# yamatokataoka/reinforcement-learning-replications

Measured on NVIDIA H100. Metric: ppo_update_transitions_per_sec, higher is better.
Workload: dtype f32

## Files before the change

### reinforcement-learning-replications_b200/csrc/mlp_tc3.cu

```cuda
#include <cuda_fp16.h>

#include <cmath>

#include "common.cuh"
#include "policy_head.cuh"
#include "tc2_common.cuh"
#include "tc_common.cuh"
#include "tc3.cuh"

namespace b200rl {

constexpr int T3_ROWS = 128;
constexpr int T3_CHAIN_WARPS = 8;
constexpr int T3_THREADS = T3_CHAIN_WARPS * 32 + 256;
constexpr int T3_WARPS = T3_THREADS / 32;

constexpr uint32_t S3_XB = 0;
constexpr uint32_t S3_H1 = 2 * T2_ACT;
constexpr uint32_t S3_H2 = S3_H1 + 2 * T2_ACT;
constexpr uint32_t S3_DZ2 = S3_H2 + 2 * T2_ACT;
constexpr uint32_t S3_DZ1 = S3_DZ2 + 2 * T2_ACT;
constexpr uint32_t T3_W1T = 32 * 128, T3_W2 = 64 * 128, T3_W3 = 16 * 128;
constexpr uint32_t S3_DO = S3_DZ1 + 2 * T2_ACT;
constexpr uint32_t S3_W = S3_DO + T2_ACT;
constexpr uint32_t S3_WNET = 2 * T3_W1T + 2 * T3_W2 + 2 * T3_W3;
constexpr uint32_t S3_OPERANDS_END = S3_W + S3_WNET;
constexpr uint32_t S3_BIAS = S3_OPERANDS_END;
constexpr uint32_t S3_DIST = S3_BIAS + 2 * 640;
constexpr uint32_t S3_SCALE = S3_DIST + 256;
constexpr uint32_t S3_XS = S3_SCALE + 128;
constexpr uint32_t S3_ADV = S3_XS + 256;
constexpr uint32_t S3_RED = S3_ADV + 16;
constexpr uint32_t S3_BARS = S3_RED + 4 * 8 * T3_WARPS;
constexpr uint32_t T3_LI_IN = 15 * T3_ROWS, T3_LI_OLD = 16 * T3_ROWS;
constexpr uint32_t T3_LI_BYTES = 17 * T3_ROWS * 4;
constexpr uint32_t S3_LOSS = S3_BARS + 128;
constexpr uint32_t S3_TOTAL = S3_LOSS + 2 * T3_LI_BYTES;
constexpr uint32_t T3_SMEM_BYTES = S3_TOTAL + 1024;
static_assert(T3_SMEM_BYTES <= 227 * 1024, "mlp_tc3 shared memory");
constexpr uint32_t S3_END_DB3 = 0;
constexpr uint32_t S3_END_SC = 1024;

constexpr uint32_t ACC_GRAD_NET = 176;
constexpr uint32_t ACC_DB3 = 2 * ACC_GRAD_NET;
static_assert(ACC_DB3 + 4 * 16 <= ACC_COLS, "mlp_tc3 accumulator columns");
constexpr uint32_t ACC_DW2 = 0, ACC_DB2 = 64, ACC_DW1 = 80, ACC_DW3 = 144;

__device__ __forceinline__ uint32_t grad_acc_off(uint32_t pcol, int n, int row, int col) {
  const int rr = row & 63;
  const int t = 32 * (rr >> 4) + 4 * (rr & 7) + ((col >> 1) & 3);
  const int e = 2 * ((rr >> 3) & 1) + (col & 1);
  return pcol * ACC_LANES + (uint32_t)((row >> 6) * 64 * n + 4 * (128 * (col >> 3) + t) + e);
}

#ifdef B200RL_TC3_TIMING
__device__ unsigned long long g_tc3_t[64];
#endif

enum { C3_G = 0, C3_U1, C3_U2, C3_U3, C3_UH2, C3_UH1, C3_W1, C3_W2, C3_W3, C3_OW3, C3_OW2, C3_OW1, C3_OB, C3_N };

__device__ __forceinline__ void mbar_arrive_expect_tx(uint32_t bar, uint32_t bytes) {
  asm volatile("mbarrier.arrive.expect_tx.shared::cta.b64 _, [%0], %1;" ::"r"(bar), "r"(bytes) : "memory");
}
__device__ __forceinline__ void bulk_copy_g2s(uint32_t dst_smem, const void* src, uint32_t bytes, uint32_t bar) {
  asm volatile("cp.async.bulk.shared::cluster.global.mbarrier::complete_tx::bytes [%0], [%1], %2, [%3];" ::"r"(dst_smem),
               "l"(src), "r"(bytes), "r"(bar)
               : "memory");
}

__global__ void __launch_bounds__(128) pack_obs_kernel(const float* __restrict__ obs, long long n_rows, int n_in,
                                                       const float* __restrict__ absmax, uint8_t* __restrict__ ximg,
                                                       float* __restrict__ xscale, float* __restrict__ bad_flag) {
  __shared__ float s_xs[32];
  const int r = threadIdx.x;
  bool bad = false;
  if (r < 32) {
    const int e = r < n_in ? fit_exp(__ldg(absmax + r), bad) : 0;
    s_xs[r] = pow2i(e);
    if (blockIdx.x == 0) {
      xscale[r] = pow2i(e);
      xscale[32 + r] = pow2i(-e);
    }
  }
  __syncthreads();
  const long long tiles = (n_rows + T3_ROWS - 1) / T3_ROWS;
  for (long long t = blockIdx.x; t < tiles; t += gridDim.x) {
    const long long row = t * T3_ROWS + r;
    float x[32];
#pragma unroll
    for (int c = 0; c < 32; ++c) x[c] = 0.f;
    if (row < n_rows) {
      const float* src = obs + row * n_in;
      float rmax = 0.f, probe = 0.f;
#pragma unroll
      for (int c = 0; c < 31; ++c)
        if (c < n_in) {
          x[c] = __ldg(src + c) * s_xs[c];
          rmax = fmaxf(rmax, fabsf(x[c]));
          probe += x[c];
        }
      if (!(rmax <= T2_RANGE) || probe != probe) bad = true;
      if (rmax > 0.f && rmax < 0.03125f) bad = true;
      x[31] = 1.0f;
    }
    uint4 h[4], l[4];
#pragma unroll
    for (int j = 0; j < 4; ++j) {
      split2h(x[8 * j + 0], x[8 * j + 1], h[j].x, l[j].x);
      split2h(x[8 * j + 2], x[8 * j + 3], h[j].y, l[j].y);
      split2h(x[8 * j + 4], x[8 * j + 5], h[j].z, l[j].z);
      split2h(x[8 * j + 6], x[8 * j + 7], h[j].w, l[j].w);
    }
    uint8_t* dst = ximg + (size_t)t * T2_ACT + (size_t)r * 128;
#pragma unroll
    for (int j = 0; j < 4; ++j) {
      *reinterpret_cast<uint4*>(dst + ((j ^ (r & 7)) << 4)) = h[j];
      *reinterpret_cast<uint4*>(dst + (((4 + j) ^ (r & 7)) << 4)) = l[j];
    }
  }
  if (bad) *bad_flag = 1.0f;
}

template <int N, int TA, int TB, int TERMS, int KSTEPS>
__device__ __forceinline__ void wg_mma(float (&d)[N / 2], const uint32_t (&alo)[TERMS], const uint32_t (&blo)[TERMS],
                                       uint32_t a_hi, uint32_t b_hi, uint32_t a_k, uint32_t b_k, uint32_t accumulate) {
  wgmma_fence();
#pragma unroll
  for (int s = 0; s < TERMS; ++s)
#pragma unroll
    for (int k = 0; k < KSTEPS; ++k)
      wgmma_run<N, TA, TB>(d, ((uint64_t)a_hi << 32) | (alo[s] + (uint32_t)k * a_k),
                           ((uint64_t)b_hi << 32) | (blo[s] + (uint32_t)k * b_k), s == 0 && k == 0 ? accumulate : 1u);
  wgmma_commit();
  wgmma_wait_all();
}
template <int N, int TB, int KSTEPS>
__device__ __forceinline__ void chain_mma(float (&d)[N / 2], const Op2 a, const Op2 b) {
  const uint32_t alo[3] = {a.lo, a.lo + a.split_step, a.lo}, blo[3] = {b.lo + b.split_step, b.lo, b.lo};
#pragma unroll
  for (int i = 0; i < N / 2; ++i) d[i] = 0.f;
  wg_mma<N, K_MAJOR, TB, 3, KSTEPS>(d, alo, blo, a.hi, b.hi, a.k_step, b.k_step, 0u);
}
__device__ __forceinline__ void stmatrix_x4(uint32_t addr, const uint32_t (&r)[4]) {
  asm volatile("stmatrix.sync.aligned.m8n8.x4.shared.b16 [%0], {%1, %2, %3, %4};" ::"r"(addr), "r"(r[0]), "r"(r[1]),
               "r"(r[2]), "r"(r[3])
               : "memory");
}
__device__ __forceinline__ void ldmatrix_x4(uint32_t addr, uint32_t (&r)[4]) {
  asm volatile("ldmatrix.sync.aligned.m8n8.x4.shared.b16 {%0, %1, %2, %3}, [%4];"
               : "=r"(r[0]), "=r"(r[1]), "=r"(r[2]), "=r"(r[3])
               : "r"(addr)
               : "memory");
}
__device__ __forceinline__ float* grad_frag(float* acc_cta, uint32_t pcol) {
  const int t = (int)(threadIdx.x & 127u);
  return acc_cta + grad_acc_off(pcol, 0, 16 * (t >> 5) + ((t & 31) >> 2), 2 * (t & 3));
}
template <int N, int KSTEPS, int TERMS>
__device__ __forceinline__ void grad_products(float (&d)[N / 2], uint32_t a_lo, const Op2 a, const Op2 b, bool first) {
  uint32_t b_lo = b.lo;
  asm volatile("" : "+r"(a_lo), "+r"(b_lo));
#pragma unroll
  for (int s = 0; s < TERMS; ++s)
#pragma unroll
    for (int k = 0; k < KSTEPS; ++k)
      wgmma_run<N, MN_MAJOR, MN_MAJOR>(d, ((uint64_t)a.hi << 32) | (a_lo + (uint32_t)k * a.k_step),
                                       ((uint64_t)b.hi << 32) | (b_lo + (s + 1 < TERMS ? b.split_step : 0u) +
                                                                 (uint32_t)k * b.k_step),
                                       s == 0 && k == 0 ? (first ? 0u : 1u) : 1u);
}
template <int N>
__device__ __forceinline__ void grad_store(float* acc_cta, uint32_t pcol, int h, const float (&d)[N / 2]) {
  float* const frag = grad_frag(acc_cta, pcol) + 64 * N * h;
#pragma unroll
  for (int j = 0; j < N / 8; ++j)
    *reinterpret_cast<float4*>(frag + 512 * j) = make_float4(d[4 * j], d[4 * j + 1], d[4 * j + 2], d[4 * j + 3]);
}

__global__ void __launch_bounds__(T3_THREADS, 1) mlp_tc3_kernel(const Tc3Args p) {
  extern __shared__ uint8_t smem_raw[];
  const bool two = p.run_policy != 0 && p.run_value != 0;
  const int G = two ? (int)(gridDim.x >> 1) : (int)gridDim.x;
  const int c = two ? (int)blockIdx.x / G : (p.run_policy != 0 ? 0 : 1);
  const int slot = (int)blockIdx.x - c * (two ? G : 0);
  const bool run_p = p.run_policy != 0 && (p.stop_flag == nullptr || *p.stop_flag == 0);
  const bool run_v = p.run_value != 0;
  if (!(c == 0 ? run_p : run_v)) return;
  if (*p.x_bad != 0.f) return;
  const int tid = threadIdx.x, lane = tid & 31;
  float* const acc = p.acc_mem + (size_t)slot * ACC_CTA_FLOATS;
  const int warp = __shfl_sync(0xffffffffu, tid >> 5, 0);
  const uint32_t raw = smem_u32(smem_raw);
  const uint32_t base = (raw + 1023u) & ~1023u;
  uint8_t* sm = smem_raw + (base - raw);
  float* s_bias = reinterpret_cast<float*>(sm + S3_BIAS);
  float* s_dist = reinterpret_cast<float*>(sm + S3_DIST);
  float* s_scale = reinterpret_cast<float*>(sm + S3_SCALE);
  float* s_xs = reinterpret_cast<float*>(sm + S3_XS);
  float* s_adv = reinterpret_cast<float*>(sm + S3_ADV);
  float* s_red = reinterpret_cast<float*>(sm + S3_RED);
  int* s_bad = reinterpret_cast<int*>(sm + S3_BARS + 120);
  const uint32_t bars = base + S3_BARS;
  const int n_in = p.n_in;
  bool bad = false;
#ifdef B200RL_TC3_TIMING
  unsigned long long tacc[64];
  for (int i = 0; i < 64; ++i) tacc[i] = 0;
  const long long t_kernel0 = clock64();
#endif

  for (uint32_t i = S3_W / 16 + tid; i < S3_OPERANDS_END / 16; i += T3_THREADS) reinterpret_cast<uint4*>(sm)[i] = make_uint4(0, 0, 0, 0);
  if (tid == 0) {
    *s_bad = 0;
    float adv_mean, adv_std;
    adv_mean_std(p.adv_stats, adv_mean, adv_std);
    s_adv[0] = adv_mean;
    s_adv[1] = 1.f / adv_std;
  }
  if (tid < 64) s_xs[tid] = __ldg(p.xscale + tid);
  float* s_par = reinterpret_cast<float*>(sm + S3_H1);
  static_assert(S3_W - S3_H1 >= 4 * (2 * 6000 + 64), "parameter staging area");
#pragma unroll 1
  for (int net = 0; net < 2; ++net) {
    const float* par = p.params[net];
    float* dst = s_par + (net == 0 ? 0 : p.P[0]);
#pragma unroll 8
    for (int i = tid; i < p.P[net]; i += T3_THREADS) dst[i] = (*(par + i));
  }
  __syncthreads();
#pragma unroll 1
  for (int net = 0; net < 2; ++net) {
    const Tc3Net& nn = p.net[net];
    const float* par = s_par + (net == 0 ? 0 : p.P[0]);
    float m1 = 0.f, m2 = 0.f, m3 = 0.f;
    for (int idx = tid; idx < nn.h1 * n_in; idx += T3_THREADS) {
      const float w = (*(par + nn.w_off[0] + idx)) * s_xs[32 + idx % n_in];
      m1 = fmaxf(m1, fabsf(w));
      if (w != w) bad = true;
    }
    for (int idx = tid; idx < nn.h2 * nn.h1; idx += T3_THREADS) {
      const float w = (*(par + nn.w_off[1] + idx));
      m2 = fmaxf(m2, fabsf(w));
      if (w != w) bad = true;
    }
    for (int idx = tid; idx < nn.n_out * nn.h2; idx += T3_THREADS) {
      const float w = (*(par + nn.w_off[2] + idx));
      m3 = fmaxf(m3, fabsf(w));
      if (w != w) bad = true;
    }
#pragma unroll
    for (int o = 16; o > 0; o >>= 1) {
      m1 = fmaxf(m1, __shfl_xor_sync(0xffffffffu, m1, o));
      m2 = fmaxf(m2, __shfl_xor_sync(0xffffffffu, m2, o));
      m3 = fmaxf(m3, __shfl_xor_sync(0xffffffffu, m3, o));
    }
    if (lane == 0) {
      s_red[warp * 8 + 4 * net + 0] = m1;
      s_red[warp * 8 + 4 * net + 1] = m2;
      s_red[warp * 8 + 4 * net + 2] = m3;
    }
  }
  __syncthreads();
  if (bad) *s_bad = 1;
  bad = false;
  if (tid < 2) {
    const int net = tid;
    const Tc3Net& nn = p.net[net];
    float m1 = 0.f, m2 = 0.f, m3 = 0.f;
    for (int w = 0; w < T3_WARPS; ++w) {
      m1 = fmaxf(m1, s_red[w * 8 + 4 * net + 0]);
      m2 = fmaxf(m2, s_red[w * 8 + 4 * net + 1]);
      m3 = fmaxf(m3, s_red[w * 8 + 4 * net + 2]);
    }
    bool b0 = false;
    const int ew1 = fit_exp(m1, b0), ew2 = fit_exp(m2, b0), ew3 = fit_exp(m3, b0);
    float typ;
    if (net == 1) {
      const float tm = __ldg(p.target_absmax);
      typ = (tm > 0.f && tm < INFINITY) ? 0.25f * tm : 1.f;
    } else if (p.dist == B200RL_DIST_GAUSSIAN) {
      float smin = INFINITY;
      for (int a = 0; a < nn.n_out; ++a) smin = fminf(smin, expf(__ldg(p.log_std + a)));
      typ = (smin > 0.f && smin < INFINITY) ? 1.f / smin : 1.f;
    } else {
      typ = 0.5f;
    }
    int eg = 3 + ilogbf(p.n_glob_f) - ilogbf(typ);
    eg = eg < -100 ? -100 : (eg > 100 ? 100 : eg);
    float* sc = s_scale + 16 * net;
    sc[C3_G] = pow2i(eg);
    sc[C3_U1] = pow2i(-ew1);
    sc[C3_U2] = pow2i(-(T2_H_EXP + ew2));
    sc[C3_U3] = pow2i(-(T2_H_EXP + ew3));
    sc[C3_UH2] = pow2i(-ew3);
// ... 29 lines not shown
        put(wb + 2 * T3_W1T, T3_W2, idx / nn.h1, idx % nn.h1, (*(par + nn.w_off[1] + idx)) * sw2);
      for (int idx = tid; idx < nn.n_out * nn.h2; idx += T3_THREADS)
        put(wb + 2 * T3_W1T + 2 * T3_W2, T3_W3, idx / nn.h2, idx % nn.h2, (*(par + nn.w_off[2] + idx)) * sw3);
    }
    float* bb = s_bias + 160 * net;
    for (int i = tid; i < 64; i += T3_THREADS) {
      bb[i] = i < nn.h1 ? (*(par + nn.b_off[0] + i)) : 0.f;
      bb[64 + i] = i < nn.h2 ? (*(par + nn.b_off[1] + i)) : 0.f;
      if (!(fabsf(bb[i]) < INFINITY) || !(fabsf(bb[64 + i]) < INFINITY)) bad = true;
    }
    for (int i = tid; i < 16; i += T3_THREADS) {
      bb[128 + i] = i < nn.n_out ? (*(par + nn.b_off[2] + i)) : 0.f;
      if (!(fabsf(bb[128 + i]) < INFINITY)) bad = true;
    }
  }
  if (p.dist == B200RL_DIST_GAUSSIAN)
    for (int a = tid; a < p.net[0].n_out; a += T3_THREADS) {
      const NormalConsts nc = normal_consts(p.log_std, a);
      s_dist[a] = nc.var;
      s_dist[16 + a] = nc.log_scale;
      s_dist[32 + a] = nc.inv_2var;
      s_dist[48 + a] = nc.inv_var;
    }
  if (bad) *s_bad = 1;
  bad = false;
  if (tid == 0) {
    mbar_init(bars + 0, 1);
    mbar_init(bars + 8, 1);
    for (int i = 0; i < 3; ++i) {
      mbar_init(bars + 16 + 8 * i, 2);
      mbar_init(bars + 40 + 8 * i, 2);
    }
    fence_mbar_init();
  }
  fence_proxy_async_smem();
  __syncthreads();

  const long long num_tiles = (p.n_rows + T3_ROWS - 1) / T3_ROWS;
  const int cta_tiles = (int)((num_tiles - slot + G - 1) / G);

  constexpr int K = K_MAJOR, MN = MN_MAJOR;
  const uint32_t ub = base;
  auto bar_ready = [&](int s) { return bars + 16u + 8u * (uint32_t)(s - 3); };
  auto bar_done = [&](int s) { return bars + 40u + 8u * (uint32_t)(s - 3); };
  double sc[5] = {0, 0, 0, 0, 0};
  int rows_done = 0;
#ifdef B200RL_TC3_TIMING
  long long t_loop0 = 0, t_loop_end = 0;
#endif

  if (warp >= T3_CHAIN_WARPS) {
    const Op2 X_M = op2_mnmajor(ub + S3_XB, T2_ACT, 64);
    const Op2 X_M16 = op2_mnmajor(ub + S3_XB + 32, T2_ACT, 64);
    const Op2 DO_M = op2_at(op2_mnmajor(ub + S3_DO, T2_ACT, 32), c * 64);
    const Op2 H1_M = op2_mnmajor(ub + S3_H1, T2_ACT, T2_ACT), H2_M = op2_mnmajor(ub + S3_H2, T2_ACT, T2_ACT);
    const Op2 DZ2_M = op2_mnmajor(ub + S3_DZ2, T2_ACT, T2_ACT), DZ1_M = op2_mnmajor(ub + S3_DZ1, T2_ACT, T2_ACT);
    const int g = (warp - T3_CHAIN_WARPS) >> 2;
    const bool producer = g == 0;
    const uint32_t ah = (uint32_t)g * (T2_ACT >> 4);
    const uint32_t gcol = c * ACC_GRAD_NET;
    float w3[16], w2[32], b2[8], w1[32];
    const uint32_t act_bytes = T3_ROWS * 4u * (uint32_t)(p.dist == B200RL_DIST_GAUSSIAN ? p.net[0].n_out : 1);
    auto load_x = [&](int k) {
      const uint32_t b = (uint32_t)(k & 1), bar = bars + 8 * b;
      const long long tile = slot + (long long)k * G;
      const size_t row0 = (size_t)tile * T3_ROWS;
      const uint32_t li = ub + S3_LOSS + b * T3_LI_BYTES;
      uint32_t e;
      asm volatile("{\n\t.reg .pred q;\n\telect.sync _|q, 0xffffffff;\n\tselp.u32 %0, 1, 0, q;\n\t}" : "=r"(e));
      if (e && (warp & 3) == 0) {
        if (c == 0) {
          mbar_arrive_expect_tx(bar, T2_ACT + act_bytes + 2 * T3_ROWS * 4);
          bulk_copy_g2s(li, reinterpret_cast<const uint8_t*>(p.actions) + (size_t)tile * act_bytes, act_bytes, bar);
          bulk_copy_g2s(li + 4 * T3_LI_IN, p.adv_raw + row0, T3_ROWS * 4, bar);
          bulk_copy_g2s(li + 4 * T3_LI_OLD, p.old_logp + row0, T3_ROWS * 4, bar);
        } else {
          mbar_arrive_expect_tx(bar, T2_ACT + T3_ROWS * 4);
          bulk_copy_g2s(li + 4 * T3_LI_IN, p.target + row0, T3_ROWS * 4, bar);
        }
        bulk_copy_g2s(ub + S3_XB + b * T2_ACT, p.ximg + (size_t)tile * T2_ACT, T2_ACT, bar);
      }
      __syncwarp();
    };
    auto release = [&](int stage) {
      wgmma_commit();
      wgmma_wait_all();
      asm volatile("bar.sync %0, 128;" ::"r"(8 + g) : "memory");
      if ((tid & 127) == 0) mbar_arrive(bar_done(stage));
    };
    if (producer && cta_tiles > 0) load_x(0);
#pragma unroll 1
    for (int k = 0; k < cta_tiles; ++k) {
      const uint32_t xo = (uint32_t)(k & 1) * T2_ACT;
      const bool first = k == 0;
      if (producer && k + 1 < cta_tiles) {
        if (k > 0) mbar_wait(bar_done(5), (uint32_t)((k - 1) & 1));
        load_x(k + 1);
      }
#ifdef B200RL_TC3_TIMING
      long long it0 = clock64(), it1;
#define TC3_GSPLIT(s)                                                   \
  it1 = clock64();                                                      \
  tacc[40 + 3 * g + (s) - 3] += (unsigned long long)(it1 - it0);
#define TC3_GEND(s)                                                     \
  it0 = clock64();                                                      \
  tacc[46 + 3 * g + (s) - 3] += (unsigned long long)(it0 - it1);
#else
#define TC3_GSPLIT(s)
#define TC3_GEND(s)
#endif
      mbar_wait(bar_ready(3), (uint32_t)(k & 1));
      TC3_GSPLIT(3)
      wgmma_fence();
      grad_products<32, 8, 1>(w3, H2_M.lo + ah, H2_M, DO_M, first);
      release(3);
      TC3_GEND(3)
      mbar_wait(bar_ready(4), (uint32_t)(k & 1));
      TC3_GSPLIT(4)
      wgmma_fence();
      grad_products<64, 8, 2>(w2, DZ2_M.lo + ah, DZ2_M, H1_M, first);
      grad_products<16, 8, 1>(b2, DZ2_M.lo + ah, DZ2_M, op2_at(X_M16, xo), first);
      release(4);
      TC3_GEND(4)
      mbar_wait(bar_ready(5), (uint32_t)(k & 1));
      TC3_GSPLIT(5)
      wgmma_fence();
      grad_products<64, 8, 1>(w1, DZ1_M.lo + ah, DZ1_M, op2_at(X_M, xo), first);
      release(5);
      TC3_GEND(5)
#undef TC3_GSPLIT
#undef TC3_GEND
    }
    if (cta_tiles > 0) {
      grad_store<32>(acc, gcol + ACC_DW3, g, w3);
      grad_store<64>(acc, gcol + ACC_DW2, g, w2);
      grad_store<16>(acc, gcol + ACC_DB2, g, b2);
      grad_store<64>(acc, gcol + ACC_DW1, g, w1);
    }
#ifdef B200RL_TC3_TIMING
    if ((tid & 127) == 0 && blockIdx.x == 0) {
      for (int s = 0; s < 3; ++s) {
        g_tc3_t[40 + 3 * g + s] = tacc[40 + 3 * g + s];
        g_tc3_t[46 + 3 * g + s] = tacc[46 + 3 * g + s];
      }
      if (producer) g_tc3_t[52] = (unsigned long long)cta_tiles;
    }
#endif
  } else {
    const int wg = warp >> 2;
    const int quad = lane >> 2, q = lane & 3;
    const int r0 = 64 * wg + 16 * (warp & 3) + quad;
    const uint32_t rows = (uint32_t)wg * (64u * 128u);
    const Op2 X_K = op2_at(op2_kmajor(ub + S3_XB, 64), rows);
    const Op2 DO_K = op2_at(op2_kmajor(ub + S3_DO, 32), rows + c * 64);
    const Op2 H1_K = op2_at(op2_kmajor(ub + S3_H1, T2_ACT), rows), H2_K = op2_at(op2_kmajor(ub + S3_H2, T2_ACT), rows);
    const Op2 DZ2_K = op2_at(op2_kmajor(ub + S3_DZ2, T2_ACT), rows);
    const Op2 W1T_M = op2_mnmajor(ub + S3_W, 32 * 128, T3_W1T);
    const Op2 W2_K = op2_kmajor(ub + S3_W + 2 * T3_W1T, T3_W2), W2_M = op2_mnmajor(ub + S3_W + 2 * T3_W1T, 64 * 128, T3_W2);
    const Op2 W3_K = op2_kmajor(ub + S3_W + 2 * T3_W1T + 2 * T3_W2, T3_W3),
              W3_M = op2_mnmajor(ub + S3_W + 2 * T3_W1T + 2 * T3_W2, 16 * 128, T3_W3);
    const float* scl = s_scale + 16 * c;
    const float* bias = s_bias + 160 * c;
    const float sH = pow2i(T2_H_EXP), hh = pow2i(-2 * T2_H_EXP);
    const int A_out = p.net[0].n_out;

    const uint32_t mat_row = base + (uint32_t)(64 * wg + 16 * (warp & 3) + 8 * ((lane >> 3) & 1) + (lane & 7)) * 128u;
    const uint32_t mat_chunk = (uint32_t)((lane >> 4) ^ (lane & 7)) << 4;
    auto mat_off = [&](uint32_t buf, int j) -> uint32_t { return mat_row + buf + (((uint32_t)j << 4) ^ mat_chunk); };
    auto store_pairs = [&](uint32_t buf, const float (&x)[32]) {
#pragma unroll
      for (int j = 0; j < 8; j += 2) {
        uint32_t h[4], l[4];
#pragma unroll
        for (int m = 0; m < 4; ++m) split2h(x[4 * j + 2 * m], x[4 * j + 2 * m + 1], h[m], l[m]);
        stmatrix_x4(mat_off(buf, j), h);
        stmatrix_x4(mat_off(buf + T2_ACT, j), l);
      }
    };
    auto act = [&](float (&z)[32], float unscale, const float* bs) {
#pragma unroll
      for (int g = 0; g < 2; ++g) {
        float t[16];
#pragma unroll
        for (int i = 0; i < 16; ++i) {
          const int e = 16 * g + i;
          t[i] = fmaf(z[e], unscale, bs[8 * (e >> 2) + 2 * q + (e & 1)]);
        }
        tanh16_scaled(t, sH);
#pragma unroll
        for (int i = 0; i < 16; ++i) z[16 * g + i] = t[i];
      }
    };
    auto dtanh = [&](float (&g)[32], float unscale, uint32_t buf) {
      const float one28 = 268435456.f;
      float m = 0.f;
#pragma unroll
      for (int j = 0; j < 8; j += 2) {
        uint32_t hw[4], lw[4];
        ldmatrix_x4(mat_off(buf, j), hw);
        ldmatrix_x4(mat_off(buf + T2_ACT, j), lw);
#pragma unroll
        for (int i = 0; i < 4; ++i) {
          const float2 a = __half22float2(*reinterpret_cast<const __half2*>(&hw[i]));
          const float2 b = __half22float2(*reinterpret_cast<const __half2*>(&lw[i]));
          const float x0 = a.x + b.x, x1 = a.y + b.y;
          float& g0 = g[4 * j + 2 * i];
          float& g1 = g[4 * j + 2 * i + 1];
          g0 = (g0 * unscale) * fmaf(-x0, x0, one28);
          g1 = (g1 * unscale) * fmaf(-x1, x1, one28);
          m = fmaxf(m, fmaxf(fabsf(g0), fabsf(g1)));
        }
      }
      if (!(m <= T2_RANGE)) bad = true;
    };
    auto wg_sync = [&]() {
      fence_proxy_async_smem();
      asm volatile("bar.sync %0, 128;" ::"r"(1 + wg) : "memory");
    };
    auto deliver = [&](int s) {
      wg_sync();
      if ((tid & 127) == 0) mbar_arrive(bar_ready(s));
    };
#ifdef B200RL_TC3_TIMING
    long long t_mark = 0;
#endif
    auto wait = [&](int s, uint32_t bar, uint32_t parity) {
#ifdef B200RL_TC3_TIMING
      const long long w0 = clock64();
#endif
      mbar_wait(bar, parity);
#ifdef B200RL_TC3_TIMING
      tacc[10 * wg + s - 1] += (unsigned long long)(clock64() - w0);
#endif
    };
    auto stage_end = [&](int s) {
#ifdef B200RL_TC3_TIMING
      const long long t = clock64();
      tacc[10 * wg + 4 + s] += (unsigned long long)(t - t_mark);
      t_mark = t;
#endif
    };

#ifdef B200RL_TC3_TIMING
    t_loop0 = clock64();
    t_mark = t_loop0;
#endif
    {
#pragma unroll 1
      for (int k = 0; k < cta_tiles; ++k) {
        const long long tile = slot + (long long)k * G;
        const uint32_t xo = (uint32_t)(k & 1) * T2_ACT;
        float d[32];
        wait(1, bars + 8 * (uint32_t)(k & 1), (uint32_t)((k >> 1) & 1));
        chain_mma<64, MN, 2>(d, op2_at(X_K, xo), W1T_M);
        act(d, scl[C3_U1], bias);
        if (k > 0) wait(1, bar_done(4), (uint32_t)((k - 1) & 1));
        store_pairs(S3_H1, d);
        wg_sync();
        stage_end(1);
        chain_mma<64, K, 4>(d, H1_K, W2_K);
        act(d, scl[C3_U2], bias + 64);
        store_pairs(S3_H2, d);
        wg_sync();
        stage_end(2);
        const int orow = r0 + 8 * q;
        const long long row = tile * T3_ROWS + orow;
        const bool owner = q < 2, valid = owner && row < p.n_rows;
        float* const s3p = acc + (ACC_DB3 + 16u * (uint32_t)((k + 2 * c) & 3)) * ACC_LANES + orow;
        float o[8];
        chain_mma<16, K, 4>(o, H2_K, W3_K);
        const float* li = reinterpret_cast<const float*>(sm + S3_LOSS + (uint32_t)(k & 1) * T3_LI_BYTES);
        float pf_act[15], pf_in = 0.f, pf_old = 0.f;
#pragma unroll
        for (int a = 0; a < 15; ++a) pf_act[a] = 0.f;
        if (valid) {
          if (c == 0) {
            if (p.dist == B200RL_DIST_GAUSSIAN) {
#pragma unroll
              for (int a = 0; a < 15; ++a)
                if (a < A_out) pf_act[a] = li[orow * A_out + a];
            } else {
              pf_act[0] = li[orow];
            }
            pf_old = li[T3_LI_OLD + orow];
          }
          pf_in = li[T3_LI_IN + orow];
        }
        float out[16];
#pragma unroll
        for (int j = 0; j < 2; ++j)
#pragma unroll
          for (int qq = 0; qq < 4; ++qq)
#pragma unroll
            for (int e = 0; e < 2; ++e) {
              const float v0 = __shfl_sync(0xffffffffu, o[4 * j + e], (lane & ~3) | qq);
              const float v1 = __shfl_sync(0xffffffffu, o[4 * j + 2 + e], (lane & ~3) | qq);
              out[8 * j + 2 * qq + e] = q == 0 ? v0 : v1;
            }
        float x0[8], x1[8];
#pragma unroll
        for (int j = 0; j < 8; ++j) x0[j] = x1[j] = 0.f;
        if (owner) {
          const float u3 = scl[C3_U3], sG = scl[C3_G];
          if (c == 0) {
            float dout[16];
#pragma unroll
            for (int a = 0; a < 16; ++a) {
              out[a] = fmaf(out[a], u3, bias[128 + a]);
              dout[a] = 0.f;
            }
            if (valid) {
              float lp, ent, dlp[16];
#pragma unroll
              for (int a = 0; a < 16; ++a) dlp[a] = 0.f;
              if (p.dist == B200RL_DIST_GAUSSIAN)
                gaussian_logp<15>(pf_act, out, s_dist + 16, VarRecip{s_dist + 48, s_dist + 32}, A_out, lp, ent, dlp);
              else
                categorical_logp<15>(out, (int)pf_act[0], A_out, lp, ent, dlp);
              const float adv = (pf_in - s_adv[0]) * s_adv[1];
              float coef;
              const float term = policy_loss(B200RL_LOSS_PPO_CLIP, lp, pf_old, adv, p.inv_n, p.clip_lo, p.clip_hi, coef);
#pragma unroll
              for (int a = 0; a < 15; ++a) dout[a] = coef * dlp[a];
              add_policy_row_sums(sc, term, lp, ent, pf_old, true);
            }
#pragma unroll
            for (int a = 0; a < 15; ++a) s3p[a * ACC_LANES] = (k >= 4 ? s3p[a * ACC_LANES] : 0.f) + dout[a];
#pragma unroll
            for (int j = 0; j < 8; ++j) {
              x0[j] = dout[j] * sG;
              x1[j] = j < 7 ? dout[8 + j] * sG : 0.f;
            }
          } else {
            float s3 = k >= 4 ? s3p[15 * ACC_LANES] : 0.f;
            if (valid) {
              float dout;
              sc[0] += (double)value_mse(fmaf(out[0], u3, bias[128]), pf_in, p.inv_n, dout);
              s3 += dout;
              x0[0] = dout * sG;
            }
            s3p[15 * ACC_LANES] = s3;
          }
          if (out_of_range8(x0) || out_of_range8(x1)) bad = true;
        }
        if (owner) {
          uint4 h0, l0, h1, l1;
          split2h(x0[0], x0[1], h0.x, l0.x);
          split2h(x0[2], x0[3], h0.y, l0.y);
          split2h(x0[4], x0[5], h0.z, l0.z);
          split2h(x0[6], x0[7], h0.w, l0.w);
          split2h(x1[0], x1[1], h1.x, l1.x);
          split2h(x1[2], x1[3], h1.y, l1.y);
          split2h(x1[4], x1[5], h1.z, l1.z);
          split2h(x1[6], x1[7], h1.w, l1.w);
          uint8_t* rowp = sm + S3_DO + (uint32_t)orow * 128u;
          const uint32_t sw = (uint32_t)(orow & 7), c4 = 4u * (uint32_t)c;
          *reinterpret_cast<uint4*>(rowp + (((c4 + 0u) ^ sw) << 4)) = h0;
          *reinterpret_cast<uint4*>(rowp + (((c4 + 1u) ^ sw) << 4)) = h1;
          *reinterpret_cast<uint4*>(rowp + (((c4 + 2u) ^ sw) << 4)) = l0;
          *reinterpret_cast<uint4*>(rowp + (((c4 + 3u) ^ sw) << 4)) = l1;
        }
        deliver(3);
        stage_end(3);
        chain_mma<64, MN, 1>(d, DO_K, W3_M);
        dtanh(d, scl[C3_UH2] * hh, S3_H2);
        store_pairs(S3_DZ2, d);
        deliver(4);
        stage_end(4);
        chain_mma<64, MN, 4>(d, DZ2_K, W2_M);
        dtanh(d, scl[C3_UH1] * hh, S3_H1);
        if (k > 0) wait(5, bar_done(5), (uint32_t)((k - 1) & 1));
        store_pairs(S3_DZ1, d);
        deliver(5);
        stage_end(5);
      }
    }
#ifdef B200RL_TC3_TIMING
    t_loop_end = clock64();
    if ((tid & 127) == 0 && blockIdx.x == 0)
      for (int i = 0; i < 10; ++i) g_tc3_t[10 * wg + i] = tacc[10 * wg + i];
#endif
    if (c == 0 && q < 2)
      for (int k = 0; k < cta_tiles; ++k) rows_done += (slot + (long long)k * G) * T3_ROWS + r0 + 8 * q < p.n_rows;
  }

  asm volatile("bar.sync 7, %0;" ::"n"(T3_THREADS) : "memory");
  {
    const int qw = warp & 3, part = warp >> 2;
    const int r = 32 * qw + lane;
    float* dst_row = p.partials + ((size_t)slot * 2 + (qw >> 1)) * (size_t)(p.P[0] + p.P[1]);
    const int m = 32 * (qw & 1) + lane;
    float v[16], w[16];
    const Tc3Net& nn = p.net[c];
    float* dst = dst_row + (c == 0 ? 0 : p.P[0]);
    const float* scn = s_scale + 16 * c;
    const bool have = cta_tiles > 0;
    const uint32_t gcol = c * ACC_GRAD_NET;
#pragma unroll 1
    for (int jb = part; jb < 8; jb += 4) {
      const uint32_t pcol = gcol + (jb < 4 ? ACC_DW2 : (jb < 6 ? ACC_DW1 : (jb == 6 ? ACC_DW3 : ACC_DB2)));
      const int pn = jb < 6 ? 64 : (jb == 6 ? 32 : 16);
      const int col = jb < 4 ? 16 * jb : (jb < 6 ? 16 * (jb - 4) : 0);
      const int col2 = jb < 4 ? col : (jb < 6 ? col + 32 : (jb == 6 ? 16 : col));
      if (have) {
#pragma unroll
        for (int j = 0; j < 16; ++j) {
          v[j] = acc[grad_acc_off(pcol, pn, r, col) + grad_acc_off(0, pn, 0, j)];
          w[j] = acc[grad_acc_off(pcol, pn, r, col2) + grad_acc_off(0, pn, 0, j)];
        }
      } else {
#pragma unroll
        for (int j = 0; j < 16; ++j) v[j] = w[j] = 0.f;
      }
      if (jb < 4) {
        const float u = scn[C3_OW2];
        if (m < nn.h2)
#pragma unroll
          for (int j = 0; j < 16; ++j)
            if (16 * jb + j < nn.h1) dst[nn.w_off[1] + m * nn.h1 + 16 * jb + j] = v[j] * u;
      } else if (jb < 6) {
        const int c0 = 16 * (jb - 4);
        const float u = scn[C3_OW1];
        if (m < nn.h1) {
#pragma unroll
          for (int j = 0; j < 16; ++j)
            if (c0 + j < n_in)
              dst[nn.w_off[0] + m * n_in + c0 + j] = ((v[j] + w[j]) * u) * s_xs[32 + c0 + j];
          if (jb == 5) dst[nn.b_off[0] + m] = (v[15] + w[15]) * scn[C3_OB];
        }
      } else if (jb == 6) {
        const float u = scn[C3_OW3];
        if (m < nn.h2)
#pragma unroll
          for (int a = 0; a < 15; ++a)
            if (a < nn.n_out) dst[nn.w_off[2] + a * nn.h2 + m] = (v[a] + w[a]) * u;
      } else {
        if (m < nn.h2) dst[nn.b_off[1] + m] = v[15] * scn[C3_OB];
      }
    }
  }
  float* e_db3 = reinterpret_cast<float*>(sm + S3_XB + S3_END_DB3);
  double* e_sc = reinterpret_cast<double*>(sm + S3_XB + S3_END_SC);
  {
    const int m = warp >> 2, rr = 32 * (warp & 3) + lane;
#pragma unroll
    for (int a = 0; a < 16; ++a) {
      const int cn = a == 15 ? 1 : 0;
      const bool have = cn == c && ((m - 2 * cn) & 3) < cta_tiles;
      float t = have ? acc[(ACC_DB3 + 16 * m + a) * ACC_LANES + rr] : 0.f;
#pragma unroll
      for (int o2 = 16; o2 > 0; o2 >>= 1) t += __shfl_xor_sync(0xffffffffu, t, o2);
      if (lane == 0) e_db3[warp * 16 + a] = t;
    }
  }
#pragma unroll
  for (int kk = 0; kk < 5; ++kk) {
    const double t = warp_sum(sc[kk]);
    if (lane == 0) e_sc[warp * 8 + kk] = t;
  }
  {
    const double t = warp_sum((double)rows_done);
    if (lane == 0) e_sc[warp * 8 + 5] = t;
  }
  __syncthreads();
  const size_t Ptot = (size_t)(p.P[0] + p.P[1]);
  if (tid < 16) {
    const int cn = tid == 15 ? 1 : 0, a = tid == 15 ? 0 : tid;
    if (cn == c && a < p.net[cn].n_out) {
      float t = 0.f;
      for (int w = 0; w < T3_WARPS; ++w) t += e_db3[w * 16 + tid];
      const size_t off = (cn == 0 ? 0 : (size_t)p.P[0]) + p.net[cn].b_off[2] + a;
      p.partials[((size_t)slot * 2) * Ptot + off] = t;
      p.partials[((size_t)slot * 2 + 1) * Ptot + off] = 0.f;
    }
  }
  const bool other_runs = c == 0 ? run_v : run_p;
  if (tid >= 32 && tid < 32 + 2 * B200RL_N_SCALARS && ((tid - 32) / B200RL_N_SCALARS == c || !other_runs)) {
    const int s = tid - 32;
    double t = 0.0;
    if (s / B200RL_N_SCALARS == c) {
      if (s < 6) {
        for (int w = 0; w < T3_CHAIN_WARPS; ++w) t += e_sc[w * 8 + s];
      } else if (s == 8) {
        for (int w = 0; w < T3_CHAIN_WARPS; ++w) t += e_sc[w * 8 + 0];
      }
    }
    p.scalar_partials[((size_t)slot * 2) * (2 * B200RL_N_SCALARS) + s] = t;
    p.scalar_partials[((size_t)slot * 2 + 1) * (2 * B200RL_N_SCALARS) + s] = 0.0;
  }
  if (bad) *s_bad = 1;
#ifdef B200RL_TC3_TIMING
  if (tid == 0 && blockIdx.x == 0) {
    g_tc3_t[53] = (unsigned long long)(t_loop0 - t_kernel0);
    g_tc3_t[54] = (unsigned long long)(t_loop_end - t_loop0);
    g_tc3_t[55] = (unsigned long long)(clock64() - t_loop_end);
  }
#endif

  __syncthreads();
  if (tid == 0 && *s_bad != 0) *p.status = 1.0f;
}

constexpr int RA3_WARPS = 8;

template <typename Acc>
__device__ __forceinline__ Acc ra3_gather(float* const* peers, int world, long long offset) {
  float x[RA3_MAX_WORLD];
#pragma unroll
  for (int r = 0; r < RA3_MAX_WORLD; ++r) {
    x[r] = 0.f;
    if (r < world) asm volatile("ld.relaxed.sys.global.f32 %0, [%1];" : "=f"(x[r]) : "l"(peers[r] + offset) : "memory");
  }
  Acc t = (Acc)0;
#pragma unroll
  for (int r = 0; r < RA3_MAX_WORLD; ++r)
    if (r < world) t += (Acc)x[r];
  return t;
}

__global__ void __launch_bounds__(RA3_WARPS * 32, 3) reduce_adam3_kernel(const Ra3Args a) {
  __shared__ float part[RA3_WARPS][32];
  __shared__ double spart[RA3_WARPS * 4][2 * B200RL_N_SCALARS];
  __shared__ double s_scal[2 * B200RL_N_SCALARS];
  const int lane = threadIdx.x & 31, warp = threadIdx.x >> 5;
  const long long Ptot = a.P[0] + a.P[1];
// ... 226 lines not shown
```

### reinforcement-learning-replications_b200/csrc/tc_common.cuh

```cuda
#pragma once
#include <cstdint>

namespace b200rl {

__device__ __forceinline__ uint32_t smem_u32(const void* p) {
  return static_cast<uint32_t>(__cvta_generic_to_shared(p));
}

__device__ __forceinline__ void mbar_init(uint32_t bar, uint32_t count) {
  asm volatile("mbarrier.init.shared::cta.b64 [%0], %1;" ::"r"(bar), "r"(count) : "memory");
}
__device__ __forceinline__ void fence_mbar_init() {
  asm volatile("fence.mbarrier_init.release.cluster;" ::: "memory");
}
__device__ __forceinline__ void mbar_arrive(uint32_t bar) {
  asm volatile("mbarrier.arrive.shared::cta.b64 _, [%0];" ::"r"(bar) : "memory");
}
__device__ __forceinline__ void mbar_wait(uint32_t bar, uint32_t parity) {
  uint32_t done = 0;
#pragma unroll 1
  for (uint32_t it = 0; it < (1u << 22); ++it) {
    asm volatile(
        "{\n\t"
        ".reg .pred p;\n\t"
        "mbarrier.try_wait.parity.shared::cta.b64 p, [%1], %2, %3;\n\t"
        "selp.u32 %0, 1, 0, p;\n\t"
        "}"
        : "=r"(done)
        : "r"(bar), "r"(parity), "r"(4000u)
        : "memory");
    if (done) return;
  }
  __trap();
}

__device__ __forceinline__ void fence_proxy_async_smem() { asm volatile("fence.proxy.async.shared::cta;" ::: "memory"); }

constexpr uint32_t ACC_COLS = 512, ACC_LANES = 128;
constexpr size_t ACC_CTA_FLOATS = (size_t)ACC_COLS * ACC_LANES;


template <int N>
__device__ __forceinline__ void acc_ld(const float* acc, int row, uint32_t col, float (&v)[N]) {
  const float* p = acc + col * ACC_LANES + row;
#pragma unroll
  for (int j = 0; j < N; ++j) v[j] = p[j * ACC_LANES];
}
template <int N>
__device__ __forceinline__ void acc_st(float* acc, int row, uint32_t col, const float (&v)[N]) {
  float* p = acc + col * ACC_LANES + row;
#pragma unroll
  for (int j = 0; j < N; ++j) p[j * ACC_LANES] = v[j];
}

__device__ __forceinline__ void acc_commit(uint32_t bar) {
  __threadfence_block();
  asm volatile("bar.sync 8, 128;" ::: "memory");
  if ((threadIdx.x & 127u) == 0) mbar_arrive(bar);
}

__host__ __device__ constexpr uint64_t make_smem_desc_sw128(uint32_t addr_bytes, uint32_t lbo_bytes,
                                                            uint32_t sbo_bytes) {
  return (uint64_t)((addr_bytes >> 4) & 0x3FFFu) | ((uint64_t)((lbo_bytes >> 4) & 0x3FFFu) << 16) |
         ((uint64_t)((sbo_bytes >> 4) & 0x3FFFu) << 32) | (1ull << 62);
}

struct Op2 {
  uint32_t lo, hi, split_step, k_step;
};
__device__ __forceinline__ Op2 op2_kmajor(uint32_t addr, uint32_t split_bytes) {
  const uint64_t d = make_smem_desc_sw128(addr, 16, 1024);
  return Op2{(uint32_t)d, (uint32_t)(d >> 32), split_bytes >> 4, 32u >> 4};
}
__device__ __forceinline__ Op2 op2_mnmajor(uint32_t addr, uint32_t atom_stride, uint32_t split_bytes) {
  const uint64_t d = make_smem_desc_sw128(addr, atom_stride, 1024);
  return Op2{(uint32_t)d, (uint32_t)(d >> 32), split_bytes >> 4, 2048u >> 4};
}
__device__ __forceinline__ Op2 op2_at(Op2 o, uint32_t byte_off) {
  o.lo += byte_off >> 4;
  return o;
}

template <int TA, int TB>
__device__ __forceinline__ void wgmma_f16_n16(float (&d)[8], uint64_t a, uint64_t b, uint32_t scale_d) {
  asm volatile(
      "{\n\t.reg .pred p;\n\tsetp.ne.b32 p, %10, 0;\n\t"
      "wgmma.mma_async.sync.aligned.m64n16k16.f32.f16.f16 {%0,%1,%2,%3,%4,%5,%6,%7}, %8, %9, p, 1, 1, %11, %12;\n\t}"
      : "+f"(d[0]), "+f"(d[1]), "+f"(d[2]), "+f"(d[3]), "+f"(d[4]), "+f"(d[5]), "+f"(d[6]), "+f"(d[7])
      : "l"(a), "l"(b), "r"(scale_d), "n"(TA), "n"(TB)
      : "memory");
}
template <int TA, int TB>
__device__ __forceinline__ void wgmma_f16_n32(float (&d)[16], uint64_t a, uint64_t b, uint32_t scale_d) {
  asm volatile(
      "{\n\t.reg .pred p;\n\tsetp.ne.b32 p, %18, 0;\n\t"
      "wgmma.mma_async.sync.aligned.m64n32k16.f32.f16.f16 {%0,%1,%2,%3,%4,%5,%6,%7,%8,%9,%10,%11,%12,%13,%14,%15}, %16, %17, p, 1, 1, %19, %20;\n\t}"
      : "+f"(d[0]), "+f"(d[1]), "+f"(d[2]), "+f"(d[3]), "+f"(d[4]), "+f"(d[5]), "+f"(d[6]), "+f"(d[7]), "+f"(d[8]), "+f"(d[9]), "+f"(d[10]), "+f"(d[11]), "+f"(d[12]), "+f"(d[13]), "+f"(d[14]), "+f"(d[15])
      : "l"(a), "l"(b), "r"(scale_d), "n"(TA), "n"(TB)
      : "memory");
}
template <int TA, int TB>
__device__ __forceinline__ void wgmma_f16_n48(float (&d)[24], uint64_t a, uint64_t b, uint32_t scale_d) {
  asm volatile(
      "{\n\t.reg .pred p;\n\tsetp.ne.b32 p, %26, 0;\n\t"
      "wgmma.mma_async.sync.aligned.m64n48k16.f32.f16.f16 {%0,%1,%2,%3,%4,%5,%6,%7,%8,%9,%10,%11,%12,%13,%14,%15,%16,%17,%18,%19,%20,%21,%22,%23}, %24, %25, p, 1, 1, %27, %28;\n\t}"
      : "+f"(d[0]), "+f"(d[1]), "+f"(d[2]), "+f"(d[3]), "+f"(d[4]), "+f"(d[5]), "+f"(d[6]), "+f"(d[7]), "+f"(d[8]), "+f"(d[9]), "+f"(d[10]), "+f"(d[11]), "+f"(d[12]), "+f"(d[13]), "+f"(d[14]), "+f"(d[15]), "+f"(d[16]), "+f"(d[17]), "+f"(d[18]), "+f"(d[19]), "+f"(d[20]), "+f"(d[21]), "+f"(d[22]), "+f"(d[23])
      : "l"(a), "l"(b), "r"(scale_d), "n"(TA), "n"(TB)
      : "memory");
}
template <int TA, int TB>
__device__ __forceinline__ void wgmma_f16_n64(float (&d)[32], uint64_t a, uint64_t b, uint32_t scale_d) {
  asm volatile(
      "{\n\t.reg .pred p;\n\tsetp.ne.b32 p, %34, 0;\n\t"
      "wgmma.mma_async.sync.aligned.m64n64k16.f32.f16.f16 {%0,%1,%2,%3,%4,%5,%6,%7,%8,%9,%10,%11,%12,%13,%14,%15,%16,%17,%18,%19,%20,%21,%22,%23,%24,%25,%26,%27,%28,%29,%30,%31}, %32, %33, p, 1, 1, %35, %36;\n\t}"
      : "+f"(d[0]), "+f"(d[1]), "+f"(d[2]), "+f"(d[3]), "+f"(d[4]), "+f"(d[5]), "+f"(d[6]), "+f"(d[7]), "+f"(d[8]), "+f"(d[9]), "+f"(d[10]), "+f"(d[11]), "+f"(d[12]), "+f"(d[13]), "+f"(d[14]), "+f"(d[15]), "+f"(d[16]), "+f"(d[17]), "+f"(d[18]), "+f"(d[19]), "+f"(d[20]), "+f"(d[21]), "+f"(d[22]), "+f"(d[23]), "+f"(d[24]), "+f"(d[25]), "+f"(d[26]), "+f"(d[27]), "+f"(d[28]), "+f"(d[29]), "+f"(d[30]), "+f"(d[31])
      : "l"(a), "l"(b), "r"(scale_d), "n"(TA), "n"(TB)
      : "memory");
}

__device__ __forceinline__ void wgmma_fence() { asm volatile("wgmma.fence.sync.aligned;" ::: "memory"); }
__device__ __forceinline__ void wgmma_commit() { asm volatile("wgmma.commit_group.sync.aligned;" ::: "memory"); }
__device__ __forceinline__ void wgmma_wait_all() { asm volatile("wgmma.wait_group.sync.aligned 0;" ::: "memory"); }

template <int N, int TA, int TB>
__device__ __forceinline__ void wgmma_run(float (&d)[N / 2], uint64_t a, uint64_t b, uint32_t scale_d) {
  if constexpr (N == 16) wgmma_f16_n16<TA, TB>(d, a, b, scale_d);
  else if constexpr (N == 32) wgmma_f16_n32<TA, TB>(d, a, b, scale_d);
  else if constexpr (N == 48) wgmma_f16_n48<TA, TB>(d, a, b, scale_d);
  else wgmma_f16_n64<TA, TB>(d, a, b, scale_d);
}

constexpr int K_MAJOR = 0, MN_MAJOR = 1;

template <int N, int TA, int TB, int T>
__device__ __forceinline__ void mma_product(float* acc_cta, uint32_t acc_col, const uint32_t (&alo)[T],
                                            const uint32_t (&blo)[T], int terms, uint32_t a_hi, uint32_t b_hi,
                                            uint32_t a_k, uint32_t b_k, int ksteps, bool acc_first) {
  static_assert(N == 16 || N == 32 || N == 48 || N == 64, "wgmma shape without a wrapper");
  const int t = (int)(threadIdx.x & 127u), w = t >> 5, l = t & 31;
  const uint32_t a_half = TA == MN_MAJOR ? ((alo[0] >> 16) & 0x3FFFu) : (64u * 128u) >> 4;
  float* acc = acc_cta + acc_col * ACC_LANES;
#pragma unroll 1
  for (int h = 0; h < 2; ++h) {
    const int m0 = 16 * w + (l >> 2) + 64 * h;
    float* frag = acc + 2 * (l & 3) * ACC_LANES + m0;
    float d[N / 2];
#pragma unroll
    for (int i = 0; i < N / 2; ++i)
      d[i] = acc_first ? frag[(8 * (i >> 2) + (i & 1)) * ACC_LANES + 8 * ((i >> 1) & 1)] : 0.f;
    wgmma_fence();
    uint32_t scale = acc_first ? 1u : 0u;
#pragma unroll
    for (int s = 0; s < T; ++s) {
      if (s >= terms) break;
      uint32_t a = alo[s] + (uint32_t)h * a_half, b = blo[s];
#pragma unroll 1
      for (int k = 0; k < ksteps; ++k) {
        wgmma_run<N, TA, TB>(d, ((uint64_t)a_hi << 32) | a, ((uint64_t)b_hi << 32) | b, scale);
        scale = 1u;
        a += a_k;
        b += b_k;
      }
    }
    wgmma_commit();
    wgmma_wait_all();
#pragma unroll
    for (int i = 0; i < N / 2; ++i) frag[(8 * (i >> 2) + (i & 1)) * ACC_LANES + 8 * ((i >> 1) & 1)] = d[i];
  }
}

}
```

Baseline: 14.49 million.

## Feed chained wgmma A operands from registers instead of shared memory

Adds register-sourced A-operand wgmma wrappers and uses them for the forward hidden-layer chain and the backward dz chains. The activations are split into fp16 hi/lo pairs kept in registers, so the dependent MMAs no longer wait for the stmatrix stores and a warpgroup barrier. Stores to shared memory still happen for the other consumers and are overlapped with the MMAs, with barrier delivery moved after the MMA issue. The risk is higher register pressure and a fragile match between the register fragment layout and what wgmma expects.

Result: faster. 15.57 million (median of 6 runs) (+7.5%).

```diff
diff --git a/reinforcement-learning-replications_b200/csrc/mlp_tc3.cu b/reinforcement-learning-replications_b200/csrc/mlp_tc3.cu
--- a/reinforcement-learning-replications_b200/csrc/mlp_tc3.cu
+++ b/reinforcement-learning-replications_b200/csrc/mlp_tc3.cu
@@ -140,6 +140,22 @@
 #pragma unroll
   for (int i = 0; i < N / 2; ++i) d[i] = 0.f;
   wg_mma<N, K_MAJOR, TB, 3, KSTEPS>(d, alo, blo, a.hi, b.hi, a.k_step, b.k_step, 0u);
+}
+template <int N, int TB, int KSTEPS>
+__device__ __forceinline__ void chain_mma_rs(float (&d)[N / 2], const uint32_t (&ah)[KSTEPS][4],
+                                             const uint32_t (&al)[KSTEPS][4], const Op2 b) {
+#pragma unroll
+  for (int i = 0; i < N / 2; ++i) d[i] = 0.f;
+  wgmma_fence();
+  auto desc = [&](uint32_t lo) { return ((uint64_t)b.hi << 32) | lo; };
+#pragma unroll
+  for (int k = 0; k < KSTEPS; ++k)
+    wgmma_run_rs<N, TB>(d, ah[k], desc(b.lo + b.split_step + (uint32_t)k * b.k_step), k == 0 ? 0u : 1u);
+#pragma unroll
+  for (int k = 0; k < KSTEPS; ++k) wgmma_run_rs<N, TB>(d, al[k], desc(b.lo + (uint32_t)k * b.k_step), 1u);
+#pragma unroll
+  for (int k = 0; k < KSTEPS; ++k) wgmma_run_rs<N, TB>(d, ah[k], desc(b.lo + (uint32_t)k * b.k_step), 1u);
+  wgmma_commit();
 }
 __device__ __forceinline__ void stmatrix_x4(uint32_t addr, const uint32_t (&r)[4]) {
   asm volatile("stmatrix.sync.aligned.m8n8.x4.shared.b16 [%0], {%1, %2, %3, %4};" ::"r"(addr), "r"(r[0]), "r"(r[1]),
@@ -475,9 +491,6 @@
     const int r0 = 64 * wg + 16 * (warp & 3) + quad;
     const uint32_t rows = (uint32_t)wg * (64u * 128u);
     const Op2 X_K = op2_at(op2_kmajor(ub + S3_XB, 64), rows);
-    const Op2 DO_K = op2_at(op2_kmajor(ub + S3_DO, 32), rows + c * 64);
-    const Op2 H1_K = op2_at(op2_kmajor(ub + S3_H1, T2_ACT), rows), H2_K = op2_at(op2_kmajor(ub + S3_H2, T2_ACT), rows);
-    const Op2 DZ2_K = op2_at(op2_kmajor(ub + S3_DZ2, T2_ACT), rows);
     const Op2 W1T_M = op2_mnmajor(ub + S3_W, 32 * 128, T3_W1T);
     const Op2 W2_K = op2_kmajor(ub + S3_W + 2 * T3_W1T, T3_W2), W2_M = op2_mnmajor(ub + S3_W + 2 * T3_W1T, 64 * 128, T3_W2);
     const Op2 W3_K = op2_kmajor(ub + S3_W + 2 * T3_W1T + 2 * T3_W2, T3_W3),
@@ -490,14 +503,18 @@
     const uint32_t mat_row = base + (uint32_t)(64 * wg + 16 * (warp & 3) + 8 * ((lane >> 3) & 1) + (lane & 7)) * 128u;
     const uint32_t mat_chunk = (uint32_t)((lane >> 4) ^ (lane & 7)) << 4;
     auto mat_off = [&](uint32_t buf, int j) -> uint32_t { return mat_row + buf + (((uint32_t)j << 4) ^ mat_chunk); };
-    auto store_pairs = [&](uint32_t buf, const float (&x)[32]) {
-#pragma unroll
-      for (int j = 0; j < 8; j += 2) {
-        uint32_t h[4], l[4];
-#pragma unroll
-        for (int m = 0; m < 4; ++m) split2h(x[4 * j + 2 * m], x[4 * j + 2 * m + 1], h[m], l[m]);
-        stmatrix_x4(mat_off(buf, j), h);
-        stmatrix_x4(mat_off(buf + T2_ACT, j), l);
+    uint32_t ph[4][4], pl[4][4];
+    auto split_pairs = [&](const float (&x)[32]) {
+#pragma unroll
+      for (int s = 0; s < 4; ++s)
+#pragma unroll
+        for (int m = 0; m < 4; ++m) split2h(x[8 * s + 2 * m], x[8 * s + 2 * m + 1], ph[s][m], pl[s][m]);
+    };
+    auto store_pairs = [&](uint32_t buf) {
+#pragma unroll
+      for (int s = 0; s < 4; ++s) {
+        stmatrix_x4(mat_off(buf, 2 * s), ph[s]);
+        stmatrix_x4(mat_off(buf + T2_ACT, 2 * s), pl[s]);
       }
     };
     auto act = [&](float (&z)[32], float unscale, const float* bs) {
@@ -536,12 +553,9 @@
       }
       if (!(m <= T2_RANGE)) bad = true;
     };
-    auto wg_sync = [&]() {
+    auto deliver = [&](int s) {
       fence_proxy_async_smem();
       asm volatile("bar.sync %0, 128;" ::"r"(1 + wg) : "memory");
-    };
-    auto deliver = [&](int s) {
-      wg_sync();
       if ((tid & 127) == 0) mbar_arrive(bar_ready(s));
     };
 #ifdef B200RL_TC3_TIMING
@@ -577,21 +591,23 @@
         wait(1, bars + 8 * (uint32_t)(k & 1), (uint32_t)((k >> 1) & 1));
         chain_mma<64, MN, 2>(d, op2_at(X_K, xo), W1T_M);
         act(d, scl[C3_U1], bias);
+        split_pairs(d);
         if (k > 0) wait(1, bar_done(4), (uint32_t)((k - 1) & 1));
-        store_pairs(S3_H1, d);
-        wg_sync();
+        store_pairs(S3_H1);
         stage_end(1);
-        chain_mma<64, K, 4>(d, H1_K, W2_K);
+        chain_mma_rs<64, K, 4>(d, ph, pl, W2_K);
+        wgmma_wait_all();
         act(d, scl[C3_U2], bias + 64);
-        store_pairs(S3_H2, d);
-        wg_sync();
+        split_pairs(d);
+        store_pairs(S3_H2);
         stage_end(2);
         const int orow = r0 + 8 * q;
         const long long row = tile * T3_ROWS + orow;
         const bool owner = q < 2, valid = owner && row < p.n_rows;
         float* const s3p = acc + (ACC_DB3 + 16u * (uint32_t)((k + 2 * c) & 3)) * ACC_LANES + orow;
         float o[8];
-        chain_mma<16, K, 4>(o, H2_K, W3_K);
+        chain_mma_rs<16, K, 4>(o, ph, pl, W3_K);
+        wgmma_wait_all();
         const float* li = reinterpret_cast<const float*>(sm + S3_LOSS + (uint32_t)(k & 1) * T3_LI_BYTES);
         float pf_act[15], pf_in = 0.f, pf_old = 0.f;
 #pragma unroll
@@ -683,17 +699,27 @@
           *reinterpret_cast<uint4*>(rowp + (((c4 + 2u) ^ sw) << 4)) = l0;
           *reinterpret_cast<uint4*>(rowp + (((c4 + 3u) ^ sw) << 4)) = l1;
         }
-        deliver(3);
-        stage_end(3);
-        chain_mma<64, MN, 1>(d, DO_K, W3_M);
+        __syncwarp();
+        {
+          uint32_t doh[1][4], dol[1][4];
+          ldmatrix_x4(mat_off(S3_DO, 4 * c), doh[0]);
+          ldmatrix_x4(mat_off(S3_DO, 4 * c + 2), dol[0]);
+          chain_mma_rs<64, MN, 1>(d, doh, dol, W3_M);
+          deliver(3);
+          stage_end(3);
+          wgmma_wait_all();
+        }
         dtanh(d, scl[C3_UH2] * hh, S3_H2);
-        store_pairs(S3_DZ2, d);
+        split_pairs(d);
+        store_pairs(S3_DZ2);
+        chain_mma_rs<64, MN, 4>(d, ph, pl, W2_M);
         deliver(4);
         stage_end(4);
-        chain_mma<64, MN, 4>(d, DZ2_K, W2_M);
+        wgmma_wait_all();
         dtanh(d, scl[C3_UH1] * hh, S3_H1);
         if (k > 0) wait(5, bar_done(5), (uint32_t)((k - 1) & 1));
-        store_pairs(S3_DZ1, d);
+        split_pairs(d);
+        store_pairs(S3_DZ1);
         deliver(5);
         stage_end(5);
       }
diff --git a/reinforcement-learning-replications_b200/csrc/tc_common.cuh b/reinforcement-learning-replications_b200/csrc/tc_common.cuh
--- a/reinforcement-learning-replications_b200/csrc/tc_common.cuh
+++ b/reinforcement-learning-replications_b200/csrc/tc_common.cuh
@@ -118,6 +118,25 @@
       : "memory");
 }
 
+template <int TB>
+__device__ __forceinline__ void wgmma_f16_n16_rs(float (&d)[8], const uint32_t (&a)[4], uint64_t b, uint32_t scale_d) {
+  asm volatile(
+      "{\n\t.reg .pred p;\n\tsetp.ne.b32 p, %13, 0;\n\t"
+      "wgmma.mma_async.sync.aligned.m64n16k16.f32.f16.f16 {%0,%1,%2,%3,%4,%5,%6,%7}, {%8,%9,%10,%11}, %12, p, 1, 1, %14;\n\t}"
+      : "+f"(d[0]), "+f"(d[1]), "+f"(d[2]), "+f"(d[3]), "+f"(d[4]), "+f"(d[5]), "+f"(d[6]), "+f"(d[7])
+      : "r"(a[0]), "r"(a[1]), "r"(a[2]), "r"(a[3]), "l"(b), "r"(scale_d), "n"(TB)
+      : "memory");
+}
+template <int TB>
+__device__ __forceinline__ void wgmma_f16_n64_rs(float (&d)[32], const uint32_t (&a)[4], uint64_t b, uint32_t scale_d) {
+  asm volatile(
+      "{\n\t.reg .pred p;\n\tsetp.ne.b32 p, %37, 0;\n\t"
+      "wgmma.mma_async.sync.aligned.m64n64k16.f32.f16.f16 {%0,%1,%2,%3,%4,%5,%6,%7,%8,%9,%10,%11,%12,%13,%14,%15,%16,%17,%18,%19,%20,%21,%22,%23,%24,%25,%26,%27,%28,%29,%30,%31}, {%32,%33,%34,%35}, %36, p, 1, 1, %38;\n\t}"
+      : "+f"(d[0]), "+f"(d[1]), "+f"(d[2]), "+f"(d[3]), "+f"(d[4]), "+f"(d[5]), "+f"(d[6]), "+f"(d[7]), "+f"(d[8]), "+f"(d[9]), "+f"(d[10]), "+f"(d[11]), "+f"(d[12]), "+f"(d[13]), "+f"(d[14]), "+f"(d[15]), "+f"(d[16]), "+f"(d[17]), "+f"(d[18]), "+f"(d[19]), "+f"(d[20]), "+f"(d[21]), "+f"(d[22]), "+f"(d[23]), "+f"(d[24]), "+f"(d[25]), "+f"(d[26]), "+f"(d[27]), "+f"(d[28]), "+f"(d[29]), "+f"(d[30]), "+f"(d[31])
+      : "r"(a[0]), "r"(a[1]), "r"(a[2]), "r"(a[3]), "l"(b), "r"(scale_d), "n"(TB)
+      : "memory");
+}
+
 __device__ __forceinline__ void wgmma_fence() { asm volatile("wgmma.fence.sync.aligned;" ::: "memory"); }
 __device__ __forceinline__ void wgmma_commit() { asm volatile("wgmma.commit_group.sync.aligned;" ::: "memory"); }
 __device__ __forceinline__ void wgmma_wait_all() { asm volatile("wgmma.wait_group.sync.aligned 0;" ::: "memory"); }
@@ -128,6 +147,12 @@
   else if constexpr (N == 32) wgmma_f16_n32<TA, TB>(d, a, b, scale_d);
   else if constexpr (N == 48) wgmma_f16_n48<TA, TB>(d, a, b, scale_d);
   else wgmma_f16_n64<TA, TB>(d, a, b, scale_d);
+}
+template <int N, int TB>
+__device__ __forceinline__ void wgmma_run_rs(float (&d)[N / 2], const uint32_t (&a)[4], uint64_t b, uint32_t scale_d) {
+  static_assert(N == 16 || N == 64, "register-A wgmma shape without a wrapper");
+  if constexpr (N == 16) wgmma_f16_n16_rs<TB>(d, a, b, scale_d);
+  else wgmma_f16_n64_rs<TB>(d, a, b, scale_d);
 }
 
 constexpr int K_MAJOR = 0, MN_MAJOR = 1;
```
